# francescofrontera/flink-jpmml

Measured on AMD Instinct MI355X. Metric: records/sec (whole node) on 1k-tree GBDT PMML at 1/2/4/8 MI355X; p50 latency, higher is better.
Workload: dtype fp32

## Files before the change

flink_jpmml_amd/ops/csrc/tree.hip:

```cpp
#include "tree_walk.h"

namespace pmml_tree {
namespace {
template <bool GENERAL, bool FEAT_LDS, int PILP = 8, bool MASKED = false, bool USKIP = false, bool PEEL = false,
          bool INL = false, int LTOP = 0, int NBUF = 2>
__device__ __forceinline__ void pointer_walk(const TreeArgs& a) {
  extern __shared__ __align__(16) uint32_t smem[];
  float* feat = reinterpret_cast<float*>(smem);
  float* accl = reinterpret_cast<float*>(smem + (FEAT_LDS ? a.n_feat * TB : 0));
  const int tid = threadIdx.x;
  const int2 blk = tree_block(a);
  const int row0 = blk.x * TB;
  const int split = blk.y;
  const int row = row0 + tid;
  bool row_ok = true;
  if (FEAT_LDS) row_ok = !stage_rows_own<TB>(a.X, a.n_rows, a.n_feat, a.ldx, a.prep, feat, row0);
  const float* xrow = a.X + (size_t)min(row, a.n_rows - 1) * a.ldx;
  if (!FEAT_LDS && a.prep && row < a.n_rows) {
    for (int f = 0; f < a.n_feat; ++f) {
      bool b = false;
      (void)prep_value(xrow[f], a.prep[f], &b);
      if (b) row_ok = false;
    }
  }
// ... 1014 lines not shown
      return -4;
    } else if (!feat_lds) {
      err = g ? go(tree_pointer_kernel<true, false>, lds_pw) : go(tree_pointer_kernel<false, false>, lds_pw);
    } else if (g) {
      err = (a.variant & VAR_POINTER_MASKED) ? go(tree_pointer_kernel<true, true, 8, true>, lds_pw)
                                             : go(tree_pointer_kernel<true, true>, lds_pw);
    } else {
      err = a.pilp == 2                      ? go(tree_pointer_kernel<false, true, 2>, lds_pw)
          : (a.variant & VAR_POINTER_MASKED) ? go(tree_pointer_kernel<false, true, 8, true>, lds_pw)
          : a.pilp == 16                     ? go(tree_pointer_kernel<false, true, 16>, lds_pw)
          : a.pilp == 4                      ? go(tree_pointer_kernel<false, true, 4>, lds_pw)
                                             : go(tree_pointer_kernel<false, true>, lds_pw);
    }
  }
  if (err) return err;
  if (hipGetLastError() != hipSuccess) return -7;
  if (splits > 1) {
    dim3 g2((a.n_rows + TB - 1) / TB);
    hipLaunchKernelGGL(tree_reduce_kernel, g2, dim3(TB), 0, stream, a, splits);
    if (hipGetLastError() != hipSuccess) return -8;
  }
  return 0;
}

PMML_API int pmml_tree_launch_many(hipStream_t stream, const TreeArgs* args, const int* meta, int count) {
  for (int i = 0; i < count; ++i) {
    const int* m = meta + 4 * i;
    const int rc = pmml_tree_launch(stream, args + i, m[0], m[1], m[2], m[3]);
    if (rc != 0) return ((i + 1) << 8) | (-rc & 0xFF);
  }
  return 0;
}

PMML_API int pmml_tree_grouped_args_size() { return (int)sizeof(GroupedTreeArgs); }

PMML_API int pmml_tree_reduce(hipStream_t stream, const TreeArgs* args, int splits) {
  const TreeArgs& a = *args;
  if (a.n_rows <= 0) return 0;
  if (a.C > 16 || splits < 1) return -3;
  dim3 g2((a.n_rows + TB - 1) / TB);
  hipLaunchKernelGGL(tree_reduce_kernel, g2, dim3(TB), 0, stream, a, splits);
  return hipGetLastError() == hipSuccess ? 0 : -8;
}

PMML_API int pmml_tree_launch_grouped(hipStream_t stream, const TreeArgs* host_models, int n,
                                      const GroupedTreeArgs* g, int depth, int tiles) {
  if (n <= 0 || tiles <= 0) return 0;
  if (g->n_models != n || g->F < 1) return -2;
  const TreeArgs& a0 = host_models[0];
  size_t lds = 0;
  for (int i = 0; i < n; ++i) {
    const TreeArgs& a = host_models[i];
    if ((a.variant & 3) == 0 || (a.variant & 3) != (a0.variant & 3) || a.rows_wide != a0.rows_wide ||
        a.mode != a0.mode)
      return -20;
    if (a.n_stage < 1 || a.n_stage > g->F || a.n_stage > (64 * 256) / a.rows_wide) return -4;
    if (a.C > 16) return -3;
    size_t need = 0;
    int chk = 0;
    switch (depth) {
      case 1: chk = wide_check<1>(a, need); break;
      case 2: chk = wide_check<2>(a, need); break;
      case 3: chk = wide_check<3>(a, need); break;
      case 4: chk = wide_check<4>(a, need); break;
      case 5: chk = wide_check<5>(a, need); break;
      case 6: chk = wide_check<6>(a, need); break;
      case 7: chk = wide_check<7>(a, need); break;
      case 8: chk = wide_check<8>(a, need); break;
      case 9: chk = wide_check<9>(a, need); break;
      case 10: chk = wide_check<10>(a, need); break;
      default: return -6;
    }
    if (chk) return chk;
    lds = need > lds ? need : lds;
  }
  int err = 0;
  switch (depth) {
    case 1: err = launch_grouped_d1(stream, a0, *g, tiles, lds); break;
    case 2: err = launch_grouped_d2(stream, a0, *g, tiles, lds); break;
    case 3: err = launch_grouped_d3(stream, a0, *g, tiles, lds); break;
    case 4: err = launch_grouped_d4(stream, a0, *g, tiles, lds); break;
    case 5: err = launch_grouped_d5(stream, a0, *g, tiles, lds); break;
    case 6: err = launch_grouped_d6(stream, a0, *g, tiles, lds); break;
    case 7: err = launch_grouped_d7(stream, a0, *g, tiles, lds); break;
    case 8: err = launch_grouped_d8(stream, a0, *g, tiles, lds); break;
    case 9: err = launch_grouped_d9(stream, a0, *g, tiles, lds); break;
    case 10: err = launch_grouped_d10(stream, a0, *g, tiles, lds); break;
    default: return -6;
  }
  if (err) return err;
  return hipGetLastError() == hipSuccess ? 0 : -7;
}

PMML_API int pmml_tree_general_args_size() { return (int)sizeof(GenTreeArgs); }

PMML_API int pmml_tree_general_launch(hipStream_t stream, const GenTreeArgs* args) {
  GenTreeArgs ga = *args;
  TreeArgs& a = ga.t;
  if (a.n_rows <= 0) return 0;
  if (a.C > 16) return -3;
  a.partial = nullptr;
  a.trees_per_split = a.n_trees;
  dim3 grid((a.n_rows + TB - 1) / TB);
  const bool feat_lds = a.n_feat <= 64;
  const size_t acc_lds = a.general ? (size_t)a.C * TB * 4 : 0;
  const size_t lds = (feat_lds ? (size_t)a.n_feat * TB * 4 : 0) + TB * 4 + acc_lds;
  const int err = dispatch_bool(a.general != 0, [&](auto G) {
// ... 24 lines not shown
```

flink_jpmml_amd/ops/csrc/tree_common.h:

```cpp
#pragma once
#include "epilogue.h"

namespace pmml_tree {

constexpr int TB = 256;

struct TreeArgs {
  const float* X;
  int n_rows, n_feat, ldx;
  int pad0;
  const FieldPrep* prep;
  const uint8_t* row_valid_in;
  const uint32_t* blob;
  const int* roots;
  const float* leaves;
  const int* tree_slot;
  int n_trees, rec_words, chunk_trees, P;
  int C, trees_per_split, general, variant;
  Epilogue epi;
  float* score;
  uint8_t* valid;
  float* probs;
  float* partial;
  const uint32_t* blob_nan;
  int chunk_trees_nan;
  int xcd_split;
  const float* tree_w;
  const float* acc_init;
  const int* feat_map;
  int rows_wide, mode;
  int n_stage, pilp;
  unsigned long long* prof;
  const float* rank_thr;
  const int* rank_cnt;
  int rank_stride;
  int leaf_onehot;
};
struct GroupedTreeArgs {
  const TreeArgs* models;
  const int* model_code;
  const int* row_start;
  const int* tile_start;
  const float* Xg;
  const int* perm;
  float* out_s;
  uint8_t* out_v;
  int n_models, F;
};
constexpr int VAR_NAN_FAST = 4;
constexpr int VAR_NAN_PLANES = 8;
constexpr int VAR_POINTER_REFILL = 16;
constexpr int VAR_POINTER_COMPACT = 32;
constexpr int VAR_POINTER_MASKED = 64;
constexpr int VAR_POINTER_SUPER = 128;
constexpr int VAR_POINTER_USKIP = 256;
constexpr int VAR_POINTER_PEEL = 512;
constexpr int VAR_POINTER_RANK3 = 1024;
constexpr int VAR_POINTER_INLINE = 4096;
constexpr int VAR_POINTER_LTOP = 8192;

#define PMML_TREE_DECL(D) int launch_perfect_d##D(hipStream_t st, const TreeArgs& a, dim3 grid, size_t lds); \
  int launch_grouped_d##D(hipStream_t st, const TreeArgs& a, const GroupedTreeArgs& g, int tiles, size_t lds);
PMML_TREE_DECL(1) PMML_TREE_DECL(2) PMML_TREE_DECL(3) PMML_TREE_DECL(4) PMML_TREE_DECL(5)
PMML_TREE_DECL(6) PMML_TREE_DECL(7) PMML_TREE_DECL(8) PMML_TREE_DECL(9) PMML_TREE_DECL(10)
#undef PMML_TREE_DECL

namespace {

__device__ __forceinline__ int2 tree_block(const TreeArgs& a) {
  if (a.xcd_split > 0) {
    const int L = blockIdx.x;
    return make_int2(L / a.xcd_split, L % a.xcd_split);
  }
  return make_int2(blockIdx.x, blockIdx.y);
}

__device__ __forceinline__ void finish_row(const TreeArgs& a, float acc0, const float* accl, int split,
                                           bool general, int row, bool row_ok) {
  if (row >= a.n_rows) return;
  if (a.partial) {
    const size_t stride = (size_t)a.n_rows;
    float* base = a.partial + (size_t)split * (a.C + 1) * stride;
    if (general) {
      for (int c = 0; c < a.C; ++c) base[c * stride + row] = accl[c * TB + threadIdx.x];
    } else {
      base[row] = acc0;
    }
    base[a.C * stride + row] = row_ok ? 0.f : 1.f;
    return;
  }
  if (general) {
    apply_epilogue(a.epi, [&](int c) { return accl[c * TB + threadIdx.x]; }, row_ok, row, a.n_rows, a.score,
                   a.valid, a.probs);
  } else {
    apply_epilogue(a.epi, [&](int) { return acc0; }, row_ok, row, a.n_rows, a.score, a.valid, a.probs);
  }
}

template <int DEPTH>
__device__ __forceinline__ bool null_flag(const char* rec, int dr_off) {
  constexpr int NI = (1 << DEPTH) - 1;
  return ((reinterpret_cast<const uint32_t*>(rec)[dr_off + (NI >> 5)] >> (NI & 31)) & 1u) != 0u;
}

constexpr int PREFETCH_Q = 8;

#define PF_DECL uint4 pf0, pf1, pf2, pf3, pf4, pf5, pf6, pf7;
#define PF_LOAD1(R, I, S4, LAST) R = (S4)[min((int)threadIdx.x + (I) * TB, (LAST))];
#define PF_LOAD(SRC, N16)                                                              \
  {                                                                                    \
    const uint4* s4_ = reinterpret_cast<const uint4*>(SRC);                            \
    const int last_ = (N16) > 0 ? (N16) - 1 : 0;                                      \
// ... 159 lines not shown
    const int t1 = t0 + a.chunk_trees;
    n16 = (t1 < te) ? (min(a.chunk_trees, te - t1) * rw) >> 2 : 0;
    PF_LOAD(n16 > 0 ? a.blob + (size_t)t1 * rw : a.blob, n16)
    if (missing) {
      traverse_chunk<DEPTH, GENERAL, true, ILP>(a, cur, nt, t0, feat_lane, acc, accl, poisoned);
    } else {
      traverse_chunk<DEPTH, GENERAL, false, ILP>(a, cur, nt, t0, feat_lane, acc, accl, poisoned);
    }
    PF_STORE(nxt, n16)
    __syncthreads();
  }
  finish_row(a, acc, accl, split, GENERAL, row, row_ok && !poisoned);
}

enum : int { MODE_SUM = 0, MODE_SLOT = 1, MODE_CLASS = 2, MODE_VOTE8 = 3 };
constexpr int WIDE_T = 1024;
constexpr int DYN_B = 8;
constexpr int DYN_SLOTS = 16;
constexpr int CMAX = 8;

template <int ROWS>
struct WideGeom {
  static constexpr int RS = ROWS / 32;
  static constexpr int G = 32 / RS;
  static constexpr int PS = ROWS;
};

#define PF4_DECL uint4 pq0, pq1, pq2, pq3;
#define PF4_LOAD(SRC, N16, T)                                                          \
  {                                                                                    \
    const uint4* s4_ = reinterpret_cast<const uint4*>(SRC);                            \
    const int last_ = (N16) > 0 ? (N16) - 1 : 0;                                      \
    pq0 = s4_[min((int)threadIdx.x + 0 * (T), last_)];                                 \
    pq1 = s4_[min((int)threadIdx.x + 1 * (T), last_)];                                 \
    pq2 = s4_[min((int)threadIdx.x + 2 * (T), last_)];                                 \
    pq3 = s4_[min((int)threadIdx.x + 3 * (T), last_)];                                 \
  }
#define PF4_STORE(DST, N16, T)                                                         \
  {                                                                                    \
    uint4* d4_ = reinterpret_cast<uint4*>(DST);                                        \
    const int i0_ = (int)threadIdx.x;                                                  \
    if (i0_ < (N16)) d4_[i0_] = pq0;                                                   \
    if (i0_ + (T) < (N16)) d4_[i0_ + (T)] = pq1;                                       \
    if (i0_ + 2 * (T) < (N16)) d4_[i0_ + 2 * (T)] = pq2;                               \
    if (i0_ + 3 * (T) < (N16)) d4_[i0_ + 3 * (T)] = pq3;                               \
  }

__host__ __device__ constexpr int perfect_rec_words(int depth, int P) {
  return ((2 * ((1 << depth) - 1) + (1 << depth) * P + ((1 << depth) - 1 + 31) / 32) + 3) & ~3;
}
__host__ __device__ constexpr int perfect_rec_words8(int depth) {
  return ((2 * ((1 << depth) - 1) + ((1 << depth) - 1 + 31) / 32) + 3) & ~3;
}

template <bool VC>
__device__ __forceinline__ float leaf_pair_select(uint32_t meta, bool right) {
  if constexpr (VC) return __uint_as_float(1u << (8u * ((meta >> (right ? 24 : 16)) & 3u)));
  const auto pr = __builtin_amdgcn_cvt_pk_f32_fp8((int)meta, true);
  return right ? pr[1] : pr[0];
}

template <int MODE>
struct WAcc;
template <>
struct WAcc<MODE_SUM> {
  float s = 0.f;
  __device__ __forceinline__ void add(const TreeArgs&, int, float v) { s += v; }
  __device__ __forceinline__ void poison() { s = __builtin_nanf(""); }
  __device__ __forceinline__ bool poisoned() const { return false; }
  __device__ __forceinline__ void finish() {}
};
template <>
struct WAcc<MODE_VOTE8> {
  uint32_t packed = 0u;
  bool pz = false;
  __device__ __forceinline__ void add(const TreeArgs&, int, float v) { packed += __float_as_uint(v); }
  __device__ __forceinline__ void poison() { pz = true; }
  __device__ __forceinline__ bool poisoned() const { return pz; }
  __device__ __forceinline__ void finish() {}
};
template <>
struct WAcc<MODE_CLASS> {
  float c[CMAX];
  bool pz = false;
  __device__ __forceinline__ WAcc() {
#pragma unroll
    for (int k = 0; k < CMAX; ++k) c[k] = 0.f;
  }
  __device__ __forceinline__ void add(const TreeArgs& a, int t, float v) {
    const float w = a.tree_w ? a.tree_w[t] : 1.f;
#pragma unroll
    for (int k = 0; k < CMAX; ++k) c[k] += (v == (float)k) ? w : 0.f;
    pz = pz || (v != v);
  }
  __device__ __forceinline__ void poison() { pz = true; }
  __device__ __forceinline__ bool poisoned() const { return pz; }
  __device__ __forceinline__ void finish() {}
};
template <>
struct WAcc<MODE_SLOT> {
  float c[CMAX];
  float run = 0.f;
  int cur = 0;
  bool pz = false;
  __device__ __forceinline__ WAcc() {
#pragma unroll
    for (int k = 0; k < CMAX; ++k) c[k] = 0.f;
  }
  __device__ __forceinline__ void flush() {
#pragma unroll
    for (int k = 0; k < CMAX; ++k) c[k] += (k == cur) ? run : 0.f;
    run = 0.f;
  }
  __device__ __forceinline__ void add(const TreeArgs& a, int t, float v) {
    const int sl = __builtin_amdgcn_readfirstlane(a.tree_slot[t]);
    if (sl != cur) {
      flush();
      cur = sl;
    }
    run += v;
  }
  __device__ __forceinline__ void poison() { pz = true; }
  __device__ __forceinline__ bool poisoned() const { return pz; }
  __device__ __forceinline__ void finish() { flush(); }
};

template <int DEPTH, bool LEAF8, bool VC = false>
__device__ __forceinline__ float walk_missing(const TreeArgs& a, const char* base, const char* feat_lane,
                                              bool& null_pred) {
  constexpr int NI = (1 << DEPTH) - 1;
  constexpr int NL = 1 << DEPTH;
  const int dr_off = LEAF8 ? 2 * NI : 2 * NI + NL;
  uint32_t j = 1u, pz = 0u;
  float lf = 0.f;
#pragma unroll
  for (int d = 0; d < DEPTH; ++d) {
    const uint2 nd = *reinterpret_cast<const uint2*>(base - 8 + (j << 3));
    const uint32_t fo = (LEAF8 && d == DEPTH - 1) ? (nd.y & 0xFFFFu) : nd.y;
    const float x = *reinterpret_cast<const float*>(feat_lane + fo);
    uint32_t right = (x >= __uint_as_float(nd.x)) ? 1u : 0u;
    const uint32_t n = j - 1u;
    const uint32_t w = reinterpret_cast<const uint32_t*>(base)[dr_off + (n >> 5)];
    const uint32_t isn = (x != x) ? 1u : 0u;
    right |= isn & (w >> (n & 31u));
    pz |= isn;
    if (LEAF8 && d == DEPTH - 1) {
      lf = leaf_pair_select<VC>(nd.y, right != 0u);
    } else {
      j = j + j + right;
    }
  }
  null_pred = pz && null_flag<DEPTH>(base, dr_off);
  return LEAF8 ? lf : (reinterpret_cast<const float*>(base + NI * 8) - NL)[j];
}

template <int DEPTH, int ILP, int G, bool LEAF8, int MODE>
__device__ __forceinline__ void traverse_chunk_g(const TreeArgs& a, const uint32_t* buf, int nt, int g, int t0,
                                                 const char* feat_lane, WAcc<MODE>& acc) {
  const int rw = a.rec_words;
  const int mt = (nt - g + G - 1) / G;
  for (int m = 0; m < mt; ++m) {
    bool nul;
    const float v = walk_missing<DEPTH, LEAF8, LEAF8 && MODE == MODE_VOTE8>(
        a, reinterpret_cast<const char*>(buf + (g + G * m) * rw), feat_lane, nul);
    if (nul) acc.poison();
    else acc.add(a, t0 + g + G * m, v);
  }
}

typedef unsigned int u32x2_t __attribute__((ext_vector_type(2)));
typedef __attribute__((address_space(3))) const u32x2_t lds_u2_t;
typedef __attribute__((address_space(3))) const float lds_f_t;
__device__ __forceinline__ uint32_t lds_addr(const void* p) {
  return (uint32_t)(uintptr_t)(__attribute__((address_space(3))) const char*)p;
}
__device__ __forceinline__ uint2 lds_ld2(uint32_t a) {
  const u32x2_t v = *(lds_u2_t*)(uintptr_t)a;
  return make_uint2(v.x, v.y);
}
__device__ __forceinline__ float lds_ldf(uint32_t a) { return *(lds_f_t*)(uintptr_t)a; }
__device__ __forceinline__ void lds_wait_all() {
  __builtin_amdgcn_sched_barrier(0);
  __builtin_amdgcn_s_waitcnt(0xC07F);
  __builtin_amdgcn_sched_barrier(0);
}

template <int DEPTH, int N, int G, bool LEAF8, bool VC = false>
__device__ __forceinline__ void fast_batch(uint32_t lds0, int g, int m, uint32_t feat_lane, float (&v)[N]) {
  constexpr int NI = (1 << DEPTH) - 1;
  constexpr int NL = 1 << DEPTH;
  constexpr uint32_t RB = 4u * (LEAF8 ? perfect_rec_words8(DEPTH) : perfect_rec_words(DEPTH, 1));
  constexpr uint32_t TS = G * RB;
  constexpr uint32_t C = 8u + 8u * NI - 4u * NL;
  const uint32_t b0 = lds0 + (uint32_t)(g + G * m) * RB;
  uint32_t k0 = 8u - b0, k1 = 16u - b0;
  __asm__("" : "+v"(k0), "+v"(k1));
  uint32_t u[N];
#pragma unroll
  for (int i = 0; i < N; ++i) {
    u[i] = b0;
    __asm__ volatile("" : "+v"(u[i]));
  }
#pragma unroll
  for (int d = 0; d + 1 < DEPTH; ++d) {
    uint2 nd[N];
#pragma unroll
    for (int i = 0; i < N; ++i) nd[i] = lds_ld2(u[i] + i * TS);
    lds_wait_all();
    float x[N];
#pragma unroll
    for (int i = 0; i < N; ++i) x[i] = lds_ldf(feat_lane + nd[i].y);
    lds_wait_all();
    uint64_t r[N];
#pragma unroll
    for (int i = 0; i < N; ++i) r[i] = __builtin_amdgcn_ballot_w64(x[i] >= __uint_as_float(nd[i].x));
    __builtin_amdgcn_sched_barrier(0);
#pragma unroll
    for (int i = 0; i < N; ++i) {
      u[i] = 2u * u[i] + (__builtin_amdgcn_inverse_ballot_w64(r[i]) ? k1 : k0);
      __asm__("" : "+v"(u[i]));
    }
  }
  uint2 nd[N], lv[N];
#pragma unroll
  for (int i = 0; i < N; ++i) {
    nd[i] = lds_ld2(u[i] + i * TS);
    if (!LEAF8) {
      uint32_t ul = u[i] + C;
      __asm__ volatile("" : "+v"(ul));
      lv[i] = lds_ld2(ul + i * TS);
    }
  }
  lds_wait_all();
  float x[N];
#pragma unroll
  for (int i = 0; i < N; ++i) x[i] = lds_ldf(feat_lane + (LEAF8 ? (nd[i].y & 0xFFFFu) : nd[i].y));
  lds_wait_all();
#pragma unroll
  for (int i = 0; i < N; ++i) {
    if (LEAF8) {
      v[i] = leaf_pair_select<VC>(nd[i].y, x[i] >= __uint_as_float(nd[i].x));
    } else {
      v[i] = (x[i] >= __uint_as_float(nd[i].x)) ? __uint_as_float(lv[i].y) : __uint_as_float(lv[i].x);
    }
  }
}

template <int DEPTH, int N, int G, bool LEAF8, int MODE>
__device__ __forceinline__ void fast_batch_acc(const TreeArgs& a, uint32_t lds0, int g, int m, int t0,
                                               uint32_t feat_lane, WAcc<MODE>& acc) {
  float v[N];
  fast_batch<DEPTH, N, G, LEAF8, LEAF8 && MODE == MODE_VOTE8>(lds0, g, m, feat_lane, v);
#pragma unroll
  for (int i = 0; i < N; ++i) acc.add(a, t0 + g + G * (m + i), v[i]);
}

template <int DEPTH, int ILP, int G, bool LEAF8, int MODE>
__device__ __forceinline__ void traverse_fast_g(const TreeArgs& a, const uint32_t* buf, int nt, int g, int t0,
                                                uint32_t feat_lane, WAcc<MODE>& acc) {
  const uint32_t lds0 = lds_addr(buf);
  const int mt = (nt - g + G - 1) / G;
  int m = 0;
  for (; m + ILP <= mt; m += ILP) fast_batch_acc<DEPTH, ILP, G, LEAF8, MODE>(a, lds0, g, m, t0, feat_lane, acc);
  if (ILP > 8 && m + 8 <= mt) {
    fast_batch_acc<DEPTH, 8, G, LEAF8, MODE>(a, lds0, g, m, t0, feat_lane, acc);
    m += 8;
  }
  if (ILP > 4 && m + 4 <= mt) {
    fast_batch_acc<DEPTH, 4, G, LEAF8, MODE>(a, lds0, g, m, t0, feat_lane, acc);
    m += 4;
  }
  if (m + 2 <= mt) {
    fast_batch_acc<DEPTH, 2, G, LEAF8, MODE>(a, lds0, g, m, t0, feat_lane, acc);
    m += 2;
  }
  if (m < mt) fast_batch_acc<DEPTH, 1, G, LEAF8, MODE>(a, lds0, g, m, t0, feat_lane, acc);
}

template <int DEPTH, int ILP, int ROWS, bool LEAF8, int MODE>
__device__ __forceinline__ void wide_tile(const TreeArgs& a, const int row0, const int split,
                                          const int* __restrict__ out_row, const bool prof_on) {
  using WG = WideGeom<ROWS>;
  constexpr int G = WG::G, RS = WG::RS, PS = WG::PS, T = WIDE_T;
  extern __shared__ __align__(16) uint32_t smem[];
  const int rw = a.rec_words;
  constexpr bool DYN = MODE == MODE_SUM && ROWS == 256;
  constexpr int NPART = DYN ? DYN_SLOTS : G;
  int* bad = reinterpret_cast<int*>(smem);
  int* any_missing = bad + ROWS;
  int* claim = bad + ROWS + 4;
  float* part = reinterpret_cast<float*>(claim + 8);
  float* feat = part + NPART * ROWS;
  const int F = a.n_stage;

  const int tid = threadIdx.x;
  const int lane = tid & 63;
  const int hw = (tid >> 6) * 2 + (lane >> 5);
  const int r_local = 32 * (hw % RS) + (lane & 31);
  const int g = __builtin_amdgcn_readfirstlane(hw / RS);
  const int tb = split * a.trees_per_split;
  const int te = min(a.n_trees, tb + a.trees_per_split);

  const unsigned long long tstart = prof_on ? __builtin_amdgcn_s_memtime() : 0ull;
  PF4_DECL
  int n16 = (tb < te) ? (min(a.chunk_trees, te - tb) * rw) >> 2 : 0;
  PF4_LOAD(n16 > 0 ? a.blob + (size_t)tb * rw : a.blob, n16, T)

  if (tid == 0) *any_missing = 0;
  if (tid < ROWS) bad[tid] = 0;
  if (tid < 8) claim[tid] = 0;
  if constexpr (DYN) {
    for (int e = tid; e < NPART * ROWS; e += T) part[e] = 0.f;
  }
  __syncthreads();
  {
    bool miss = false;
    const bool vec4 = a.feat_map == nullptr && (a.ldx & 3) == 0 && (reinterpret_cast<uintptr_t>(a.X) & 15) == 0;
    const int F4 = (F + 3) >> 2;
    for (int e = tid; vec4 && e < ROWS * F4; e += T) {
      const int q = e >> 5;
      const int rh = q / F4;
      const int fq = q - rh * F4;
      const int r = 32 * rh + (e & 31);
      const int row = row0 + r;
      float4 v = make_float4(0.f, 0.f, 0.f, 0.f);
      if (row < a.n_rows) v = *reinterpret_cast<const float4*>(a.X + (size_t)row * a.ldx + 4 * fq);
      const float vv[4] = {v.x, v.y, v.z, v.w};
      bool b = false;
#pragma unroll
      for (int k = 0; k < 4; ++k) {
        const int f = 4 * fq + k;
        if (f < F) {
          float x = vv[k];
          if (row < a.n_rows) {
            if (a.prep) x = prep_value(x, a.prep[f], &b);
            miss = miss || (x != x);
          }
          feat[f * PS + r] = x;
        }
      }
      if (b) bad[r] = 1;
    }
    const int total = vec4 ? 0 : ROWS * F;
    for (int e = tid; e < total; e += T) {
      const int q = e >> 5;
      const int rh = q / F;
      const int f = q - rh * F;
      const int r = 32 * rh + (e & 31);
      const int row = row0 + r;
      float x = 0.f;
      bool b = false;
      if (row < a.n_rows) {
        const int col = a.feat_map ? a.feat_map[f] : f;
        x = a.X[(size_t)row * a.ldx + col];
        if (a.prep) x = prep_value(x, a.prep[col], &b);
        miss = miss || (x != x);
      }
      feat[f * PS + r] = x;
      if (b) bad[r] = 1;
    }
    if (__any(miss) && lane == 0) *any_missing = 1;
  }
  __syncthreads();
  const bool has_missing = *any_missing != 0;
  const bool use_nan = has_missing && a.blob_nan != nullptr;
  const uint32_t* blob = use_nan ? a.blob_nan : a.blob;
  const int chunk = use_nan ? a.chunk_trees_nan : a.chunk_trees;
  uint32_t* tbuf0 = reinterpret_cast<uint32_t*>(feat + (use_nan ? 2 : 1) * F * PS);
  uint32_t* tbuf1 = tbuf0 + chunk * rw;
  if (use_nan) {
    const int total = PS * F;
    for (int e = tid; e < total; e += T) {
      const float x = feat[e];
      feat[total + e] = (x != x) ? __builtin_inff() : x;
    }
    n16 = (tb < te) ? (min(chunk, te - tb) * rw) >> 2 : 0;
    PF4_LOAD(n16 > 0 ? blob + (size_t)tb * rw : blob, n16, T)
  }
  PF4_STORE(tbuf0, n16, T)
  __syncthreads();

  const bool missing = has_missing && (a.variant & VAR_NAN_FAST) == 0;
  WAcc<MODE> acc;
  const char* feat_lane = reinterpret_cast<const char*>(feat + r_local);
  unsigned long long tp0 = 0, tp1 = 0, tp2 = 0, tq = 0;
  if (prof_on) tq = __builtin_amdgcn_s_memtime(), tp0 = tq - tstart;
  int c = 0;
  for (int t0 = tb; t0 < te; t0 += chunk, ++c) {
    const int nt = min(chunk, te - t0);
    const uint32_t* cur = (c & 1) ? tbuf1 : tbuf0;
    uint32_t* nxt = (c & 1) ? tbuf0 : tbuf1;
    const int t1 = t0 + chunk;
    n16 = (t1 < te) ? (min(chunk, te - t1) * rw) >> 2 : 0;
    PF4_LOAD(n16 > 0 ? blob + (size_t)t1 * rw : blob, n16, T)
    if constexpr (DYN) {
      int* ctr = claim + (c & 1) * 4 + ((tid >> 6) % (RS / 2 > 0 ? RS / 2 : 1));
      if (tid < 4) claim[((c + 1) & 1) * 4 + tid] = 0;
      const uint32_t lds0 = lds_addr(cur);
      const uint32_t fl = lds_addr(feat + r_local);
      const int nb = (nt + DYN_B - 1) / DYN_B;
      for (;;) {
        int b = 0;
        if (lane == 0) b = atomicAdd(ctr, 1);
        b = __builtin_amdgcn_readfirstlane(b);
        if (b >= nb) break;
        const int m = b * DYN_B;
        float sum = 0.f;
        if (missing) {
          const int me = min(m + DYN_B, nt);
          for (int t = m; t < me; ++t) {
            bool nul;
            const float v = walk_missing<DEPTH, LEAF8>(a, reinterpret_cast<const char*>(cur + t * rw), feat_lane, nul);
            sum += nul ? __builtin_nanf("") : v;
          }
        } else if (m + DYN_B <= nt) {
          float v[DYN_B];
          fast_batch<DEPTH, DYN_B, 1, LEAF8>(lds0, 0, m, fl, v);
#pragma unroll
          for (int i = 0; i < DYN_B; ++i) sum += v[i];
        } else {
          int mm = m;
          if (mm + 4 <= nt) {
            float v[4];
            fast_batch<DEPTH, 4, 1, LEAF8>(lds0, 0, mm, fl, v);
#pragma unroll
            for (int i = 0; i < 4; ++i) sum += v[i];
            mm += 4;
          }
          if (mm + 2 <= nt) {
            float v[2];
            fast_batch<DEPTH, 2, 1, LEAF8>(lds0, 0, mm, fl, v);
            sum += v[0];
            sum += v[1];
            mm += 2;
          }
          if (mm < nt) {
            float v[1];
            fast_batch<DEPTH, 1, 1, LEAF8>(lds0, 0, mm, fl, v);
            sum += v[0];
          }
        }
        part[(((t0 - tb) / DYN_B + b) % DYN_SLOTS) * ROWS + r_local] += sum;
      }
    } else if (missing) {
      traverse_chunk_g<DEPTH, ILP, G, LEAF8, MODE>(a, cur, nt, g, t0, feat_lane, acc);
    } else {
      traverse_fast_g<DEPTH, ILP, G, LEAF8, MODE>(a, cur, nt, g, t0, lds_addr(feat + r_local), acc);
    }
    unsigned long long tm = 0;
    if (prof_on) tm = __builtin_amdgcn_s_memtime(), tp1 += tm - tq;
    PF4_STORE(nxt, n16, T)
    __syncthreads();
    if (prof_on) tq = __builtin_amdgcn_s_memtime(), tp2 += tq - tm;
  }
  acc.finish();
  if (prof_on && lane == 0) {
    unsigned long long* pw = a.prof + (tid >> 6) * 4;
    pw[0] = tp0;
    pw[1] = tp1;
    pw[2] = tp2;
    pw[3] = __builtin_amdgcn_s_memtime() - tstart;
  }
  if (acc.poisoned()) bad[r_local] = 1;
  const int row = row0 + r_local;
  if constexpr (MODE == MODE_SUM) {
    if constexpr (!DYN) {
      part[g * ROWS + r_local] = acc.s;
      __syncthreads();
    }
    if (g == 0) {
      float sum = part[r_local];
#pragma unroll
      for (int q = 1; q < NPART; ++q) sum += part[q * ROWS + r_local];
      bool row_ok = bad[r_local] == 0;
      if (a.row_valid_in && row < a.n_rows) row_ok = row_ok && a.row_valid_in[row];
      if (row < a.n_rows) {
        if (a.partial) {
          const size_t stride = (size_t)a.n_rows;
          float* pbase = a.partial + (size_t)split * 2 * stride;
          pbase[row] = sum;
          pbase[stride + row] = row_ok ? 0.f : 1.f;
        } else {
          const int orow = out_row ? out_row[row] : row;
          apply_epilogue(a.epi, [&](int) { return sum; }, row_ok, orow, a.n_rows, a.score, a.valid, a.probs);
        }
      }
    }
  } else {
    float tot[CMAX];
#pragma unroll
    for (int k = 0; k < CMAX; ++k) tot[k] = 0.f;
    if constexpr (MODE == MODE_VOTE8) {
      reinterpret_cast<uint32_t*>(part)[g * ROWS + r_local] = acc.packed;
      __syncthreads();
      if (g == 0) {
#pragma unroll
        for (int q = 0; q < G; ++q) {
          const uint32_t pk = reinterpret_cast<const uint32_t*>(part)[q * ROWS + r_local];
#pragma unroll
          for (int k = 0; k < 4; ++k) tot[k] += (float)((pk >> (8 * k)) & 0xFFu);
        }
      }
    } else {
#pragma unroll
      for (int k = 0; k < CMAX; ++k) {
        if (k < a.C) {
          part[g * ROWS + r_local] = acc.c[k];
          __syncthreads();
          if (g == 0) {
#pragma unroll
            for (int q = 0; q < G; ++q) tot[k] += part[q * ROWS + r_local];
          }
          __syncthreads();
        }
      }
    }
    if (g == 0 && row < a.n_rows) {
      if (a.acc_init) {
#pragma unroll
        for (int k = 0; k < CMAX; ++k)
          if (k < a.C) tot[k] += a.acc_init[k];
      }
      bool row_ok = bad[r_local] == 0;
      if (a.row_valid_in) row_ok = row_ok && a.row_valid_in[row];
      auto sel = [&](int cls) {
        float r = tot[0];
#pragma unroll
        for (int k = 1; k < CMAX; ++k) r = (cls == k) ? tot[k] : r;
        return r;
      };
      apply_epilogue(a.epi, sel, row_ok, out_row ? out_row[row] : row, a.n_rows, a.score, a.valid, a.probs);
    }
  }
}

template <int DEPTH, int ILP, int ROWS, bool LEAF8, int MODE>
__global__ __launch_bounds__(WIDE_T, 1) void tree_perfect_wide_kernel(TreeArgs a) {
  const bool prof_on = a.prof != nullptr && blockIdx.x == gridDim.x / 2 && blockIdx.y == 0;
  wide_tile<DEPTH, ILP, ROWS, LEAF8, MODE>(a, blockIdx.x * ROWS, blockIdx.y, nullptr, prof_on);
}

template <int DEPTH, int ILP, int ROWS, bool LEAF8, int MODE>
__global__ __launch_bounds__(WIDE_T, 1) void tree_grouped_wide_kernel(GroupedTreeArgs ga) {
  const int t = ga.tile_start[0] + (int)blockIdx.x;
  if (t >= ga.tile_start[ga.n_models]) return;
  int lo = 0, hi = ga.n_models - 1;
  while (lo < hi) {
    const int mid = (lo + hi + 1) >> 1;
    if (ga.tile_start[mid] <= t) lo = mid;
    else hi = mid - 1;
  }
  const int e = __builtin_amdgcn_readfirstlane(lo);
  TreeArgs a = ga.models[e];
  const int code = ga.model_code[e];
  const int rs = ga.row_start[code];
  a.X = ga.Xg + (size_t)rs * ga.F;
  a.ldx = ga.F;
  a.n_feat = ga.F;
  a.n_rows = ga.row_start[code + 1] - rs;
  a.score = ga.out_s;
  a.valid = ga.out_v;
  a.row_valid_in = nullptr;
  a.partial = nullptr;
  a.prof = nullptr;
  a.trees_per_split = a.n_trees;
  wide_tile<DEPTH, ILP, ROWS, LEAF8, MODE>(a, (t - ga.tile_start[e]) * ROWS, 0, ga.perm + rs, false);
}

template <typename K>
int prepare_launch(K kernel, size_t lds) {
  if (lds > 65536) {
    hipError_t e = hipFuncSetAttribute(reinterpret_cast<const void*>(kernel),
                                       hipFuncAttributeMaxDynamicSharedMemorySize, (int)lds);
    if (e != hipSuccess) return (int)e;
  }
  return 0;
}

template <int D, int ROWS, bool LEAF8, int MODE>
int launch_wide(hipStream_t st, const TreeArgs& a, size_t lds_w) {
  using WG = WideGeom<ROWS>;
  dim3 grid((a.n_rows + ROWS - 1) / ROWS, (a.n_trees + a.trees_per_split - 1) / a.trees_per_split);
  (void)WG::G;
  auto k = tree_perfect_wide_kernel<D, 8, ROWS, LEAF8, MODE>;
  int err = prepare_launch(k, lds_w);
  if (!err) hipLaunchKernelGGL(k, grid, dim3(WIDE_T), lds_w, st, a);
  return err;
}

template <int D>
int wide_check(const TreeArgs& a, size_t& lds_w) {
  const bool leaf8 = (a.variant & 3) == 2;
  const int rows = a.rows_wide;
  if (!(rows == 256 || rows == 128 || rows == 64)) return -12;
  const int G = WIDE_T / rows;
  const bool dyn = a.mode == MODE_SUM && rows == 256;
  const int npart = dyn ? DYN_SLOTS : G;
  const size_t head = (size_t)(rows + 4 + 8) * 4 + (size_t)npart * rows * 4;
  if (dyn && (a.chunk_trees > DYN_B * DYN_SLOTS || (a.blob_nan && a.chunk_trees_nan > DYN_B * DYN_SLOTS)))
    return -14;
  const size_t plane = (size_t)a.n_stage * rows * 4;
  lds_w = head + plane + 2 * (size_t)a.chunk_trees * a.rec_words * 4;
  if ((size_t)a.chunk_trees * a.rec_words > (size_t)WIDE_T * 4 * 4) return -9;
  if (a.blob_nan) {
    if (a.chunk_trees_nan < 1 || (size_t)a.chunk_trees_nan * a.rec_words > (size_t)WIDE_T * 4 * 4) return -9;
    lds_w = max(lds_w, head + 2 * plane + 2 * (size_t)a.chunk_trees_nan * a.rec_words * 4);
  }
  if (lds_w > 160 * 1024) return -5;
  if (a.P != 1 || a.rec_words != (leaf8 ? perfect_rec_words8(D) : perfect_rec_words(D, 1))) return -10;
  if (a.mode != MODE_SUM && (a.partial || a.C > CMAX || (a.mode == MODE_VOTE8 && a.C > 4) ||
                             (leaf8 && a.mode != MODE_VOTE8)))
    return -11;
  if (a.mode == MODE_SLOT && !a.tree_slot) return -11;
  return 0;
}

template <int D>
int launch_grouped(hipStream_t st, const TreeArgs& a, const GroupedTreeArgs& g, int tiles, size_t lds) {
  const bool leaf8 = (a.variant & 3) == 2;
#define PMML_GROUPED(R, L8, M)                                                       \
  {                                                                                  \
    auto k = tree_grouped_wide_kernel<D, 8, R, L8, M>;                               \
    int err = prepare_launch(k, lds);                                                \
    if (!err) hipLaunchKernelGGL(k, dim3(tiles), dim3(WIDE_T), lds, st, g);          \
    return err;                                                                      \
  }
#define PMML_GROUPED_ROWS(R)                                                         \
  if (a.rows_wide == R) {                                                            \
    switch (a.mode) {                                                                \
      case MODE_SUM:                                                                 \
        if (leaf8) PMML_GROUPED(R, true, MODE_SUM) else PMML_GROUPED(R, false, MODE_SUM)       \
      case MODE_SLOT: PMML_GROUPED(R, false, MODE_SLOT)                              \
      case MODE_CLASS: PMML_GROUPED(R, false, MODE_CLASS)                            \
      case MODE_VOTE8:                                                               \
        if (leaf8) PMML_GROUPED(R, true, MODE_VOTE8) else PMML_GROUPED(R, false, MODE_VOTE8)   \
      default: return -11;                                                           \
    }                                                                                \
  }
  PMML_GROUPED_ROWS(256)
  PMML_GROUPED_ROWS(128)
  PMML_GROUPED_ROWS(64)
#undef PMML_GROUPED_ROWS
#undef PMML_GROUPED
  return -12;
}

template <int D>
int launch_perfect(hipStream_t st, const TreeArgs& a, dim3 grid, size_t lds) {
  int err = 0;
  const int base = a.variant & 3;
  if (base == 1 || base == 2) {
    const bool leaf8 = base == 2;
    const int rows = a.rows_wide;
    size_t lds_w = 0;
    const int chk = wide_check<D>(a, lds_w);
    if (chk) return chk;
    (void)grid;
    (void)lds;
#define PMML_WIDE_ROWS(R)                                                                     \
    if (rows == R) {                                                                          \
      switch (a.mode) {                                                                       \
        case MODE_SUM: return leaf8 ? launch_wide<D, R, true, MODE_SUM>(st, a, lds_w)         \
                                    : launch_wide<D, R, false, MODE_SUM>(st, a, lds_w);       \
        case MODE_SLOT: return launch_wide<D, R, false, MODE_SLOT>(st, a, lds_w);             \
        case MODE_CLASS: return launch_wide<D, R, false, MODE_CLASS>(st, a, lds_w);           \
        case MODE_VOTE8: return leaf8 ? launch_wide<D, R, true, MODE_VOTE8>(st, a, lds_w)     \
                                      : launch_wide<D, R, false, MODE_VOTE8>(st, a, lds_w);   \
        default: return -11;                                                                  \
      }                                                                                       \
    }
    PMML_WIDE_ROWS(256)
    PMML_WIDE_ROWS(128)
    PMML_WIDE_ROWS(64)
#undef PMML_WIDE_ROWS
    return -12;
  }
  if (base == 2 || (a.variant & ~3)) return -10;
  if (a.general) {
    err = prepare_launch(tree_perfect_kernel<D, true, 4>, lds);
    if (!err) hipLaunchKernelGGL((tree_perfect_kernel<D, true, 4>), grid, dim3(TB), lds, st, a);
  } else {
    err = prepare_launch(tree_perfect_kernel<D, false, 8>, lds);
    if (!err) hipLaunchKernelGGL((tree_perfect_kernel<D, false, 8>), grid, dim3(TB), lds, st, a);
  }
  return err;
}

}
}
```

Baseline: 439.5 million.

## Keep leaf values in global memory for dynamic wide kernel, staging only split nodes

For the dynamic-claim MODE_SUM wide path with fp32 leaves, only the split thresholds, feature indices and null flags of each tree are staged into LDS. Leaf values are now read straight from global memory at the end of each walk. The smaller LDS record lets larger chunks fit, and a new batched gather overlaps the previous batch's leaf loads with the next batch's walk. A variant flag restores the old LDS-leaf path. The cost is scattered global leaf loads and more complex waitcnt-based pipelining.

Measured after the change: 439.6 million, median of 5. No clear change (+0.0%).

```diff
diff --git a/flink_jpmml_amd/ops/csrc/tree.hip b/flink_jpmml_amd/ops/csrc/tree.hip
--- a/flink_jpmml_amd/ops/csrc/tree.hip
+++ b/flink_jpmml_amd/ops/csrc/tree.hip
@@ -1090,7 +1090,7 @@
   for (int i = 0; i < n; ++i) {
     const TreeArgs& a = host_models[i];
     if ((a.variant & 3) == 0 || (a.variant & 3) != (a0.variant & 3) || a.rows_wide != a0.rows_wide ||
-        a.mode != a0.mode)
+        a.mode != a0.mode || ((a.variant ^ a0.variant) & VAR_WIDE_LDS_LEAVES))
       return -20;
     if (a.n_stage < 1 || a.n_stage > g->F || a.n_stage > (64 * 256) / a.rows_wide) return -4;
     if (a.C > 16) return -3;
diff --git a/flink_jpmml_amd/ops/csrc/tree_common.h b/flink_jpmml_amd/ops/csrc/tree_common.h
--- a/flink_jpmml_amd/ops/csrc/tree_common.h
+++ b/flink_jpmml_amd/ops/csrc/tree_common.h
@@ -58,6 +58,7 @@
 constexpr int VAR_POINTER_RANK3 = 1024;
 constexpr int VAR_POINTER_INLINE = 4096;
 constexpr int VAR_POINTER_LTOP = 8192;
+constexpr int VAR_WIDE_LDS_LEAVES = 1 << 14;
 
 #define PMML_TREE_DECL(D) int launch_perfect_d##D(hipStream_t st, const TreeArgs& a, dim3 grid, size_t lds); \
   int launch_grouped_d##D(hipStream_t st, const TreeArgs& a, const GroupedTreeArgs& g, int tiles, size_t lds);
@@ -323,6 +324,64 @@
 __host__ __device__ constexpr int perfect_rec_words8(int depth) {
   return ((2 * ((1 << depth) - 1) + ((1 << depth) - 1 + 31) / 32) + 3) & ~3;
 }
+
+#ifndef PMML_WIDE_CHUNK_MAX
+#define PMML_WIDE_CHUNK_MAX (DYN_B * DYN_SLOTS)
+#endif
+__host__ __device__ inline int wide_chunk(const TreeArgs& a, int depth, bool nan) {
+  const int c = nan ? a.chunk_trees_nan : a.chunk_trees;
+  if (c < DYN_B || c % DYN_B != 0) return c;
+  const int head = (256 + 4 + 8) * 4 + DYN_SLOTS * 256 * 4;
+  const int plane = a.n_stage * 256 * 4;
+  int per = (160 * 1024 - head - (nan ? 2 : 1) * plane) / 2;
+  if (per > WIDE_T * 4 * 16) per = WIDE_T * 4 * 16;
+  int fit = per / (4 * perfect_rec_words8(depth));
+  if (fit > PMML_WIDE_CHUNK_MAX) fit = PMML_WIDE_CHUNK_MAX;
+  fit = fit / DYN_B * DYN_B;
+  return fit > c ? fit : c;
+}
+
+typedef unsigned int glb_u2_t __attribute__((ext_vector_type(2)));
+typedef unsigned int glb_u4_t __attribute__((ext_vector_type(4)));
+template <typename V>
+__device__ __forceinline__ V glb_ld(uint64_t addr) {
+  return *(__attribute__((address_space(1))) const V*)addr;
+}
+template <typename V>
+__device__ __forceinline__ V glb_ld(const void* p) {
+  return glb_ld<V>((uint64_t)(uintptr_t)p);
+}
+__device__ __forceinline__ uint64_t uniform64(uint64_t v) {
+  return ((uint64_t)(uint32_t)__builtin_amdgcn_readfirstlane((int)(v >> 32)) << 32) |
+         (uint32_t)__builtin_amdgcn_readfirstlane((int)(uint32_t)v);
+}
+
+template <int DEPTH>
+__device__ __forceinline__ uint4 rec8_load(const uint32_t* src, int q) {
+  constexpr int NI = (1 << DEPTH) - 1;
+  constexpr int NL = 1 << DEPTH;
+  constexpr int R4 = perfect_rec_words8(DEPTH) / 4;
+  constexpr int S4 = (2 * NI - 2) / 4;
+  const int k = q / R4;
+  const int w4 = q - k * R4;
+  const uint32_t* rec = src + (size_t)k * perfect_rec_words(DEPTH, 1);
+  if (w4 == S4) {
+    const glb_u2_t lo = glb_ld<glb_u2_t>(rec + 2 * NI - 2);
+    const glb_u2_t hi = glb_ld<glb_u2_t>(rec + 2 * NI + NL);
+    return make_uint4(lo.x, lo.y, hi.x, hi.y);
+  }
+  const glb_u4_t v = glb_ld<glb_u4_t>(rec + 4 * w4 + (w4 > S4 ? NL : 0));
+  return make_uint4(v.x, v.y, v.z, v.w);
+}
+#define PF4_LOAD_REC8(D, SRC, N16, T)                                                  \
+  {                                                                                    \
+    const uint32_t* s_ = (SRC);                                                        \
+    const int last_ = (N16) > 0 ? (N16) - 1 : 0;                                      \
+    pq0 = rec8_load<D>(s_, min((int)threadIdx.x + 0 * (T), last_));                    \
+    pq1 = rec8_load<D>(s_, min((int)threadIdx.x + 1 * (T), last_));                    \
+    pq2 = rec8_load<D>(s_, min((int)threadIdx.x + 2 * (T), last_));                    \
+    pq3 = rec8_load<D>(s_, min((int)threadIdx.x + 3 * (T), last_));                    \
+  }
 
 template <bool VC>
 __device__ __forceinline__ float leaf_pair_select(uint32_t meta, bool right) {
@@ -396,12 +455,12 @@
   __device__ __forceinline__ void finish() { flush(); }
 };
 
-template <int DEPTH, bool LEAF8, bool VC = false>
+template <int DEPTH, bool LEAF8, bool VC = false, bool GLEAF = false>
 __device__ __forceinline__ float walk_missing(const TreeArgs& a, const char* base, const char* feat_lane,
-                                              bool& null_pred) {
+                                              bool& null_pred, const uint32_t* gleaves = nullptr) {
   constexpr int NI = (1 << DEPTH) - 1;
   constexpr int NL = 1 << DEPTH;
-  const int dr_off = LEAF8 ? 2 * NI : 2 * NI + NL;
+  const int dr_off = (LEAF8 || GLEAF) ? 2 * NI : 2 * NI + NL;
   uint32_t j = 1u, pz = 0u;
   float lf = 0.f;
 #pragma unroll
@@ -422,6 +481,7 @@
     }
   }
   null_pred = pz && null_flag<DEPTH>(base, dr_off);
+  if constexpr (GLEAF) return __uint_as_float(glb_ld<uint32_t>(gleaves + (j - NL)));
   return LEAF8 ? lf : (reinterpret_cast<const float*>(base + NI * 8) - NL)[j];
 }
 
@@ -517,6 +577,74 @@
   }
 }
 
+template <int DEPTH>
+__device__ __forceinline__ uint64_t gather_base(uint64_t blob, int tree, uint32_t b0) {
+  constexpr uint32_t NL = 1u << DEPTH;
+  return blob + (uint64_t)(uint32_t)tree * (4u * perfect_rec_words(DEPTH, 1)) + 4u * NL - b0;
+}
+template <int DEPTH, int N, typename Between>
+__device__ __forceinline__ void gather_batch(uint32_t lds0, int m, uint32_t feat_lane, uint64_t blob, int tree,
+                                             float (&v)[N], Between between) {
+  constexpr uint32_t RB = 4u * perfect_rec_words8(DEPTH);
+  constexpr uint32_t RG = 4u * perfect_rec_words(DEPTH, 1);
+  const uint32_t b0 = lds0 + (uint32_t)m * RB;
+  const uint64_t gleaf = gather_base<DEPTH>(blob, tree, b0);
+  uint32_t k0 = 8u - b0, k1 = 16u - b0;
+  __asm__("" : "+v"(k0), "+v"(k1));
+  uint32_t u[N];
+#pragma unroll
+  for (int i = 0; i < N; ++i) {
+    u[i] = b0;
+    __asm__ volatile("" : "+v"(u[i]));
+  }
+  if constexpr (DEPTH == 1) between();
+#pragma unroll
+  for (int d = 0; d + 1 < DEPTH; ++d) {
+    uint2 nd[N];
+#pragma unroll
+    for (int i = 0; i < N; ++i) nd[i] = lds_ld2(u[i] + i * RB);
+    lds_wait_all();
+    float x[N];
+#pragma unroll
+    for (int i = 0; i < N; ++i) x[i] = lds_ldf(feat_lane + nd[i].y);
+    lds_wait_all();
+    uint64_t r[N];
+#pragma unroll
+    for (int i = 0; i < N; ++i) r[i] = __builtin_amdgcn_ballot_w64(x[i] >= __uint_as_float(nd[i].x));
+    __builtin_amdgcn_sched_barrier(0);
+#pragma unroll
+    for (int i = 0; i < N; ++i) {
+      u[i] = 2u * u[i] + (__builtin_amdgcn_inverse_ballot_w64(r[i]) ? k1 : k0);
+      __asm__("" : "+v"(u[i]));
+    }
+    if (d == 0) between();
+  }
+  uint2 nd[N];
+#pragma unroll
+  for (int i = 0; i < N; ++i) nd[i] = lds_ld2(u[i] + i * RB);
+  lds_wait_all();
+  float x[N];
+#pragma unroll
+  for (int i = 0; i < N; ++i) x[i] = lds_ldf(feat_lane + nd[i].y);
+  lds_wait_all();
+  uint64_t r[N];
+#pragma unroll
+  for (int i = 0; i < N; ++i) r[i] = __builtin_amdgcn_ballot_w64(x[i] >= __uint_as_float(nd[i].x));
+  __builtin_amdgcn_sched_barrier(0);
+  constexpr int PER = 4095 / (int)RG + 1;
+  uint64_t gb[(N + PER - 1) / PER];
+#pragma unroll
+  for (int q = 0; q < (N + PER - 1) / PER; ++q) {
+    gb[q] = gleaf + (uint64_t)(q * PER) * RG;
+    __asm__("" : "+s"(gb[q]));
+  }
+#pragma unroll
+  for (int i = 0; i < N; ++i) {
+    const uint32_t off = u[i] + (__builtin_amdgcn_inverse_ballot_w64(r[i]) ? 4u : 0u);
+    v[i] = __uint_as_float(glb_ld<uint32_t>(gb[i / PER] + (uint64_t)((i % PER) * RG) + (uint64_t)off));
+  }
+}
+
 template <int DEPTH, int N, int G, bool LEAF8, int MODE>
 __device__ __forceinline__ void fast_batch_acc(const TreeArgs& a, uint32_t lds0, int g, int m, int t0,
                                                uint32_t feat_lane, WAcc<MODE>& acc) {
@@ -548,7 +676,7 @@
   if (m < mt) fast_batch_acc<DEPTH, 1, G, LEAF8, MODE>(a, lds0, g, m, t0, feat_lane, acc);
 }
 
-template <int DEPTH, int ILP, int ROWS, bool LEAF8, int MODE>
+template <int DEPTH, int ILP, int ROWS, bool LEAF8, int MODE, bool LDSLEAF>
 __device__ __forceinline__ void wide_tile(const TreeArgs& a, const int row0, const int split,
                                           const int* __restrict__ out_row, const bool prof_on) {
   using WG = WideGeom<ROWS>;
@@ -557,6 +685,8 @@
   const int rw = a.rec_words;
   constexpr bool DYN = MODE == MODE_SUM && ROWS == 256;
   constexpr int NPART = DYN ? DYN_SLOTS : G;
+  constexpr bool GL = DYN && !LEAF8 && !LDSLEAF;
+  const int rl = GL ? perfect_rec_words8(DEPTH) : rw;
   int* bad = reinterpret_cast<int*>(smem);
   int* any_missing = bad + ROWS;
   int* claim = bad + ROWS + 4;
@@ -574,8 +704,12 @@
 
   const unsigned long long tstart = prof_on ? __builtin_amdgcn_s_memtime() : 0ull;
   PF4_DECL
-  int n16 = (tb < te) ? (min(a.chunk_trees, te - tb) * rw) >> 2 : 0;
-  PF4_LOAD(n16 > 0 ? a.blob + (size_t)tb * rw : a.blob, n16, T)
+  const int chunk_main = GL ? wide_chunk(a, DEPTH, false) : a.chunk_trees;
+  int n16 = (tb < te) ? (min(chunk_main, te - tb) * rl) >> 2 : 0;
+#define PF4_LOAD_CHUNK(SRC, N16)                      \
+  if constexpr (GL) PF4_LOAD_REC8(DEPTH, SRC, N16, T) \
+  else PF4_LOAD(SRC, N16, T)
+  PF4_LOAD_CHUNK(n16 > 0 ? a.blob + (size_t)tb * rw : a.blob, n16)
 
   if (tid == 0) *any_missing = 0;
   if (tid < ROWS) bad[tid] = 0;
@@ -636,17 +770,17 @@
   const bool has_missing = *any_missing != 0;
   const bool use_nan = has_missing && a.blob_nan != nullptr;
   const uint32_t* blob = use_nan ? a.blob_nan : a.blob;
-  const int chunk = use_nan ? a.chunk_trees_nan : a.chunk_trees;
+  const int chunk = use_nan ? (GL ? wide_chunk(a, DEPTH, true) : a.chunk_trees_nan) : chunk_main;
   uint32_t* tbuf0 = reinterpret_cast<uint32_t*>(feat + (use_nan ? 2 : 1) * F * PS);
-  uint32_t* tbuf1 = tbuf0 + chunk * rw;
+  uint32_t* tbuf1 = tbuf0 + chunk * rl;
   if (use_nan) {
     const int total = PS * F;
     for (int e = tid; e < total; e += T) {
       const float x = feat[e];
       feat[total + e] = (x != x) ? __builtin_inff() : x;
     }
-    n16 = (tb < te) ? (min(chunk, te - tb) * rw) >> 2 : 0;
-    PF4_LOAD(n16 > 0 ? blob + (size_t)tb * rw : blob, n16, T)
+    n16 = (tb < te) ? (min(chunk, te - tb) * rl) >> 2 : 0;
+    PF4_LOAD_CHUNK(n16 > 0 ? blob + (size_t)tb * rw : blob, n16)
   }
   PF4_STORE(tbuf0, n16, T)
   __syncthreads();
@@ -662,56 +796,122 @@
     const uint32_t* cur = (c & 1) ? tbuf1 : tbuf0;
     uint32_t* nxt = (c & 1) ? tbuf0 : tbuf1;
     const int t1 = t0 + chunk;
-    n16 = (t1 < te) ? (min(chunk, te - t1) * rw) >> 2 : 0;
-    PF4_LOAD(n16 > 0 ? blob + (size_t)t1 * rw : blob, n16, T)
+    n16 = (t1 < te) ? (min(chunk, te - t1) * rl) >> 2 : 0;
+    PF4_LOAD_CHUNK(n16 > 0 ? blob + (size_t)t1 * rw : blob, n16)
     if constexpr (DYN) {
       int* ctr = claim + (c & 1) * 4 + ((tid >> 6) % (RS / 2 > 0 ? RS / 2 : 1));
       if (tid < 4) claim[((c + 1) & 1) * 4 + tid] = 0;
-      const uint32_t lds0 = lds_addr(cur);
       const uint32_t fl = lds_addr(feat + r_local);
       const int nb = (nt + DYN_B - 1) / DYN_B;
-      for (;;) {
+      auto claim_batch = [&]() {
         int b = 0;
         if (lane == 0) b = atomicAdd(ctr, 1);
-        b = __builtin_amdgcn_readfirstlane(b);
-        if (b >= nb) break;
-        const int m = b * DYN_B;
-        float sum = 0.f;
+        return __builtin_amdgcn_readfirstlane(b);
+      };
+      auto slot_of = [&](int b) { return part + (((t0 - tb) / DYN_B + b) % DYN_SLOTS) * ROWS + r_local; };
+      if constexpr (GL) {
+        const uint32_t lds0 = (uint32_t)__builtin_amdgcn_readfirstlane((int)lds_addr(cur));
+        const uint64_t gblob = uniform64((uint64_t)(uintptr_t)blob);
         if (missing) {
-          const int me = min(m + DYN_B, nt);
-          for (int t = m; t < me; ++t) {
-            bool nul;
-            const float v = walk_missing<DEPTH, LEAF8>(a, reinterpret_cast<const char*>(cur + t * rw), feat_lane, nul);
-            sum += nul ? __builtin_nanf("") : v;
+          for (int b = claim_batch(); b < nb; b = claim_batch()) {
+            const int m = b * DYN_B, me = min(m + DYN_B, nt);
+            float sum = 0.f;
+            for (int t = m; t < me; ++t) {
+              bool nul;
+              const float v = walk_missing<DEPTH, false, false, true>(
+                  a, reinterpret_cast<const char*>(cur + t * rl), feat_lane, nul,
+                  blob + (size_t)(t0 + t) * rw + 2 * ((1 << DEPTH) - 1));
+              sum += nul ? __builtin_nanf("") : v;
+            }
+            *slot_of(b) += sum;
           }
-        } else if (m + DYN_B <= nt) {
-          float v[DYN_B];
-          fast_batch<DEPTH, DYN_B, 1, LEAF8>(lds0, 0, m, fl, v);
-#pragma unroll
-          for (int i = 0; i < DYN_B; ++i) sum += v[i];
         } else {
-          int mm = m;
-          if (mm + 4 <= nt) {
-            float v[4];
-            fast_batch<DEPTH, 4, 1, LEAF8>(lds0, 0, mm, fl, v);
-#pragma unroll
-            for (int i = 0; i < 4; ++i) sum += v[i];
-            mm += 4;
+          const int nbf = nt / DYN_B;
+          auto none = []() {};
+          int b = claim_batch();
+          if (b < nbf) {
+            float pl[DYN_B];
+            gather_batch<DEPTH, DYN_B>(lds0, b * DYN_B, fl, gblob, t0 + b * DYN_B, pl, none);
+            float* pslot = slot_of(b);
+            auto retire = [&]() {
+              __builtin_amdgcn_s_waitcnt(0x0F70);
+              float s = 0.f;
+#pragma unroll
+              for (int i = 0; i < DYN_B; ++i) s += pl[i];
+              *pslot += s;
+            };
+            for (b = claim_batch(); b < nbf; b = claim_batch()) {
+              gather_batch<DEPTH, DYN_B>(lds0, b * DYN_B, fl, gblob, t0 + b * DYN_B, pl, retire);
+              pslot = slot_of(b);
+            }
+            retire();
           }
-          if (mm + 2 <= nt) {
-            float v[2];
-            fast_batch<DEPTH, 2, 1, LEAF8>(lds0, 0, mm, fl, v);
-            sum += v[0];
-            sum += v[1];
-            mm += 2;
-          }
-          if (mm < nt) {
-            float v[1];
-            fast_batch<DEPTH, 1, 1, LEAF8>(lds0, 0, mm, fl, v);
-            sum += v[0];
+          if (b == nbf && nbf < nb) {
+            int mm = b * DYN_B;
+            float sum = 0.f;
+            if (mm + 4 <= nt) {
+              float v[4];
+              gather_batch<DEPTH, 4>(lds0, mm, fl, gblob, t0 + mm, v, none);
+#pragma unroll
+              for (int i = 0; i < 4; ++i) sum += v[i];
+              mm += 4;
+            }
+            if (mm + 2 <= nt) {
+              float v[2];
+              gather_batch<DEPTH, 2>(lds0, mm, fl, gblob, t0 + mm, v, none);
+              sum += v[0];
+              sum += v[1];
+              mm += 2;
+            }
+            if (mm < nt) {
+              float v[1];
+              gather_batch<DEPTH, 1>(lds0, mm, fl, gblob, t0 + mm, v, none);
+              sum += v[0];
+            }
+            *slot_of(b) += sum;
           }
         }
-        part[(((t0 - tb) / DYN_B + b) % DYN_SLOTS) * ROWS + r_local] += sum;
+      } else {
+        const uint32_t lds0 = lds_addr(cur);
+        for (int b = claim_batch(); b < nb; b = claim_batch()) {
+          const int m = b * DYN_B;
+          float sum = 0.f;
+          if (missing) {
+            const int me = min(m + DYN_B, nt);
+            for (int t = m; t < me; ++t) {
+              bool nul;
+              const float v = walk_missing<DEPTH, LEAF8>(a, reinterpret_cast<const char*>(cur + t * rw), feat_lane, nul);
+              sum += nul ? __builtin_nanf("") : v;
+            }
+          } else if (m + DYN_B <= nt) {
+            float v[DYN_B];
+            fast_batch<DEPTH, DYN_B, 1, LEAF8>(lds0, 0, m, fl, v);
+#pragma unroll
+            for (int i = 0; i < DYN_B; ++i) sum += v[i];
+          } else {
+            int mm = m;
+            if (mm + 4 <= nt) {
+              float v[4];
+              fast_batch<DEPTH, 4, 1, LEAF8>(lds0, 0, mm, fl, v);
+#pragma unroll
+              for (int i = 0; i < 4; ++i) sum += v[i];
+              mm += 4;
+            }
+            if (mm + 2 <= nt) {
+              float v[2];
+              fast_batch<DEPTH, 2, 1, LEAF8>(lds0, 0, mm, fl, v);
+              sum += v[0];
+              sum += v[1];
+              mm += 2;
+            }
+            if (mm < nt) {
+              float v[1];
+              fast_batch<DEPTH, 1, 1, LEAF8>(lds0, 0, mm, fl, v);
+              sum += v[0];
+            }
+          }
+          *slot_of(b) += sum;
+        }
       }
     } else if (missing) {
       traverse_chunk_g<DEPTH, ILP, G, LEAF8, MODE>(a, cur, nt, g, t0, feat_lane, acc);
@@ -805,13 +1005,13 @@
   }
 }
 
-template <int DEPTH, int ILP, int ROWS, bool LEAF8, int MODE>
+template <int DEPTH, int ILP, int ROWS, bool LEAF8, int MODE, bool LDSLEAF = false>
 __global__ __launch_bounds__(WIDE_T, 1) void tree_perfect_wide_kernel(TreeArgs a) {
   const bool prof_on = a.prof != nullptr && blockIdx.x == gridDim.x / 2 && blockIdx.y == 0;
-  wide_tile<DEPTH, ILP, ROWS, LEAF8, MODE>(a, blockIdx.x * ROWS, blockIdx.y, nullptr, prof_on);
-}
-
-template <int DEPTH, int ILP, int ROWS, bool LEAF8, int MODE>
+  wide_tile<DEPTH, ILP, ROWS, LEAF8, MODE, LDSLEAF>(a, blockIdx.x * ROWS, blockIdx.y, nullptr, prof_on);
+}
+
+template <int DEPTH, int ILP, int ROWS, bool LEAF8, int MODE, bool LDSLEAF = false>
 __global__ __launch_bounds__(WIDE_T, 1) void tree_grouped_wide_kernel(GroupedTreeArgs ga) {
   const int t = ga.tile_start[0] + (int)blockIdx.x;
   if (t >= ga.tile_start[ga.n_models]) return;
@@ -835,7 +1035,7 @@
   a.partial = nullptr;
   a.prof = nullptr;
   a.trees_per_split = a.n_trees;
-  wide_tile<DEPTH, ILP, ROWS, LEAF8, MODE>(a, (t - ga.tile_start[e]) * ROWS, 0, ga.perm + rs, false);
+  wide_tile<DEPTH, ILP, ROWS, LEAF8, MODE, LDSLEAF>(a, (t - ga.tile_start[e]) * ROWS, 0, ga.perm + rs, false);
 }
 
 template <typename K>
@@ -848,12 +1048,12 @@
   return 0;
 }
 
-template <int D, int ROWS, bool LEAF8, int MODE>
+template <int D, int ROWS, bool LEAF8, int MODE, bool LDSLEAF = false>
 int launch_wide(hipStream_t st, const TreeArgs& a, size_t lds_w) {
   using WG = WideGeom<ROWS>;
   dim3 grid((a.n_rows + ROWS - 1) / ROWS, (a.n_trees + a.trees_per_split - 1) / a.trees_per_split);
   (void)WG::G;
-  auto k = tree_perfect_wide_kernel<D, 8, ROWS, LEAF8, MODE>;
+  auto k = tree_perfect_wide_kernel<D, 8, ROWS, LEAF8, MODE, LDSLEAF>;
   int err = prepare_launch(k, lds_w);
   if (!err) hipLaunchKernelGGL(k, grid, dim3(WIDE_T), lds_w, st, a);
   return err;
@@ -871,11 +1071,15 @@
   if (dyn && (a.chunk_trees > DYN_B * DYN_SLOTS || (a.blob_nan && a.chunk_trees_nan > DYN_B * DYN_SLOTS)))
     return -14;
   const size_t plane = (size_t)a.n_stage * rows * 4;
-  lds_w = head + plane + 2 * (size_t)a.chunk_trees * a.rec_words * 4;
-  if ((size_t)a.chunk_trees * a.rec_words > (size_t)WIDE_T * 4 * 4) return -9;
+  const bool gl = dyn && !leaf8 && (a.variant & VAR_WIDE_LDS_LEAVES) == 0;
+  const size_t rl = gl ? perfect_rec_words8(D) : a.rec_words;
+  const size_t chunk = gl ? wide_chunk(a, D, false) : a.chunk_trees;
+  const size_t chunk_nan = gl ? wide_chunk(a, D, true) : a.chunk_trees_nan;
+  lds_w = head + plane + 2 * chunk * rl * 4;
+  if (chunk * rl > (size_t)WIDE_T * 4 * 4) return -9;
   if (a.blob_nan) {
-    if (a.chunk_trees_nan < 1 || (size_t)a.chunk_trees_nan * a.rec_words > (size_t)WIDE_T * 4 * 4) return -9;
-    lds_w = max(lds_w, head + 2 * plane + 2 * (size_t)a.chunk_trees_nan * a.rec_words * 4);
+    if (a.chunk_trees_nan < 1 || chunk_nan * rl > (size_t)WIDE_T * 4 * 4) return -9;
+    lds_w = max(lds_w, head + 2 * plane + 2 * chunk_nan * rl * 4);
   }
   if (lds_w > 160 * 1024) return -5;
   if (a.P != 1 || a.rec_words != (leaf8 ? perfect_rec_words8(D) : perfect_rec_words(D, 1))) return -10;
@@ -889,9 +1093,10 @@
 template <int D>
 int launch_grouped(hipStream_t st, const TreeArgs& a, const GroupedTreeArgs& g, int tiles, size_t lds) {
   const bool leaf8 = (a.variant & 3) == 2;
-#define PMML_GROUPED(R, L8, M)                                                       \
+  const bool ldsleaf = (a.variant & VAR_WIDE_LDS_LEAVES) != 0;
+#define PMML_GROUPED(R, L8, M, ...)                                                  \
   {                                                                                  \
-    auto k = tree_grouped_wide_kernel<D, 8, R, L8, M>;                               \
+    auto k = tree_grouped_wide_kernel<D, 8, R, L8, M, ##__VA_ARGS__>;                \
     int err = prepare_launch(k, lds);                                                \
     if (!err) hipLaunchKernelGGL(k, dim3(tiles), dim3(WIDE_T), lds, st, g);          \
     return err;                                                                      \
@@ -900,7 +1105,9 @@
   if (a.rows_wide == R) {                                                            \
     switch (a.mode) {                                                                \
       case MODE_SUM:                                                                 \
-        if (leaf8) PMML_GROUPED(R, true, MODE_SUM) else PMML_GROUPED(R, false, MODE_SUM)       \
+        if (leaf8) PMML_GROUPED(R, true, MODE_SUM)                                   \
+        else if (ldsleaf) PMML_GROUPED(R, false, MODE_SUM, R == 256)                 \
+        else PMML_GROUPED(R, false, MODE_SUM)                                        \
       case MODE_SLOT: PMML_GROUPED(R, false, MODE_SLOT)                              \
       case MODE_CLASS: PMML_GROUPED(R, false, MODE_CLASS)                            \
       case MODE_VOTE8:                                                               \
@@ -922,6 +1129,7 @@
   const int base = a.variant & 3;
   if (base == 1 || base == 2) {
     const bool leaf8 = base == 2;
+    const bool ldsleaf = (a.variant & VAR_WIDE_LDS_LEAVES) != 0;
     const int rows = a.rows_wide;
     size_t lds_w = 0;
     const int chk = wide_check<D>(a, lds_w);
@@ -932,7 +1140,8 @@
     if (rows == R) {                                                                          \
       switch (a.mode) {                                                                       \
         case MODE_SUM: return leaf8 ? launch_wide<D, R, true, MODE_SUM>(st, a, lds_w)         \
-                                    : launch_wide<D, R, false, MODE_SUM>(st, a, lds_w);       \
+                     : ldsleaf ? launch_wide<D, R, false, MODE_SUM, R == 256>(st, a, lds_w)    \
+                               : launch_wide<D, R, false, MODE_SUM>(st, a, lds_w);            \
         case MODE_SLOT: return launch_wide<D, R, false, MODE_SLOT>(st, a, lds_w);             \
         case MODE_CLASS: return launch_wide<D, R, false, MODE_CLASS>(st, a, lds_w);           \
         case MODE_VOTE8: return leaf8 ? launch_wide<D, R, true, MODE_VOTE8>(st, a, lds_w)     \
```
